# undistro/trivy

Hardware: AMD Instinct MI355X
Metric: GB/s secret-scanned (whole node) at 1/2/4/8 MI355X; findings bit-exact vs CPU (higher is better)
Workload: dtype u8

## Files before the change

### include/tsg_debug.h

```cpp
#ifndef TSG_DEBUG_H
#define TSG_DEBUG_H
#include <stdint.h>
#ifdef __cplusplus
extern "C" {
#endif

int tsg_regex_find_all(const char* pattern, const uint8_t* text, uint64_t n, int submatch,
                       const int64_t* windows, uint32_t n_windows, int64_t* out, uint64_t out_cap,
                       uint64_t* out_len, int32_t* num_cap);

void tsg_debug_regex_engine(int mode);
int tsg_debug_xform(int device, const uint8_t* raw, uint64_t n_bytes, const uint64_t* offsets, uint32_t n_files,
                    const uint8_t* kinds, uint8_t* out, uint64_t out_cap, uint64_t* xoff);
int tsg_debug_classify(int device, const uint8_t* raw, uint64_t n_bytes, const uint64_t* offsets, uint32_t n_files,
                       uint8_t* flags);
int tsg_debug_transform_census(int device, const uint8_t* raw, uint64_t n_bytes, const uint64_t* offsets,
                               uint32_t n_files, const uint8_t* kinds, uint8_t* mark_out);
int tsg_debug_gather_device(int device, const uint8_t* raw, uint64_t n_bytes, const uint64_t* src_off,
                            const uint64_t* dst_off, uint32_t n_files, uint8_t* out);
int tsg_regex_match(const char* pattern, const uint8_t* text, uint64_t n);

int64_t tsg_go_bytes_to_lower(const uint8_t* s, uint64_t n, uint8_t* out, uint64_t out_cap);

struct tsg_global;
// ... 20 lines not shown
                     int32_t* off_lo, int32_t* off_hi);
const char* tsg_debug_keyword(const tsg_compiled* c, uint32_t k);
const void* tsg_debug_anchor_req(const tsg_compiled* c, uint32_t j);
int tsg_debug_filter(const tsg_compiled* c, uint32_t* shape, const uint32_t** reach, const uint32_t** bucket_off,
                     const uint32_t** bucket_items, const void** items, uint32_t* n_items, const uint8_t** item_cls,
                     const uint32_t** classes, double* est_fp);
int tsg_debug_filter_ids(const tsg_compiled* c, const uint32_t** ids, uint32_t* n);
int tsg_debug_filter_core(const tsg_compiled* c, uint32_t out[4]);
const char* tsg_debug_rule_anchor(const tsg_compiled* c, uint32_t i);


int tsg_debug_pool_budget(void);

struct tsg_scanner;
int tsg_debug_scanner_engine(struct tsg_scanner* s, uint64_t out[4]);

int tsg_debug_scanner_gpu_findings(struct tsg_scanner* s, int mode);

int tsg_debug_scanner_fetch(struct tsg_scanner* s, uint64_t stage_bytes, uint64_t direct_bytes);

int tsg_regex_find_all_bounded(const char* pattern, const uint8_t* text, uint64_t true_len, uint64_t lo, uint64_t hi,
                               int submatch, const int64_t* windows, uint32_t n_windows, int64_t* out,
                               uint64_t out_cap, uint64_t* out_len, int32_t* num_cap, int32_t* hit_limit);
int tsg_debug_fetch_windows_plan(const uint64_t* offsets, uint32_t n_files, const void* cands, uint64_t n_cands,
                                 const uint32_t* rule_max_len, uint32_t n_rules, const uint32_t* opts, uint64_t* runs,
                                 uint64_t runs_cap, uint64_t* n_runs, uint64_t* views, uint64_t views_cap,
                                 uint64_t* n_views, uint64_t totals[4]);
int tsg_debug_fetch_windows_device(int device, const uint8_t* arena, uint64_t n_bytes, const uint64_t* offsets,
                                   uint32_t n_files, const void* cands, uint64_t n_cands, uint32_t cand_cap,
                                   const uint32_t* rule_max_len, uint32_t n_rules, const uint32_t* opts,
// ... 16 lines not shown
  uint32_t kw_words;
  uint32_t counters[16];
  uint32_t caps[3];
  uint32_t reserved_;
  uint64_t* hits;        uint64_t hits_cap, n_hits;
  uint32_t* kw;          uint64_t kw_cap, n_kw;
  uint32_t* flags;       uint64_t flags_cap, n_flags;
  uint16_t* nl;          uint64_t nl_cap, n_nl;
  uint32_t* chunk_file;  uint64_t chunk_file_cap, n_chunk_file;
  uint32_t* recs;        uint64_t recs_cap, n_recs;
  void* cands;           uint64_t cands_cap, n_cands;
} tsg_debug_stage_dump;
int tsg_debug_engine_stages(const tsg_compiled* c, int device, const uint8_t* arena, uint64_t n_bytes,
                            const uint64_t* offsets, uint32_t n_files, const uint8_t tail[64],
                            tsg_debug_stage_dump* out);
int tsg_debug_scan_grow(const uint32_t counters[16], const uint32_t fs_counters[6], uint32_t caps[7]);

int tsg_debug_tar_headers(int device, const void* dev_tar, uint64_t n_bytes, uint64_t capacity, uint32_t grid_cap,
                          void* records_out, uint64_t* count_out, double* ms_out);
void tsg_debug_set_tar_capacity(uint64_t records);
struct tsg_analyzer;
struct tsg_tar_index;
struct tsg_device_tar_stats;
int tsg_debug_index_tar_records(struct tsg_analyzer* a, const uint8_t* host_tar, uint64_t n_bytes,
                                const void* records, uint64_t n_records, struct tsg_tar_index** out,
                                struct tsg_device_tar_stats* st);
int tsg_debug_tar_chain(int device, const void* dev_tar, uint64_t n_bytes, uint32_t segment_blocks, uint32_t grid_cap,
                        void* records_out, uint64_t rec_cap, uint64_t* n_records, uint8_t* names_out,
                        uint64_t name_cap, uint64_t* name_bytes, uint64_t* stop_out, uint64_t* candidates_out);
int tsg_debug_tar_walk_last_fallback(const struct tsg_analyzer* a);
// ... 14 lines not shown
```

### trivy_amd/csrc/capi_debug.cpp

```cpp
#include "tsg_debug.h"

#include <algorithm>
#include <atomic>
#include <cstring>
#include <memory>
#include <string>
#include <vector>

#include "capi_internal.h"
#include "census.h"
#include "classify.h"
#include "fetch_host.h"
#include "fetch_windows.h"
#include "filter.h"
#include "goregex.h"
#include "parallel.h"
#include "xform.h"

namespace tsg {
extern std::atomic<int> g_regex_engine;
thread_local std::string g_last_error;
void SetError(const std::string& e) { g_last_error = e; }
}

extern "C" {

const char* tsg_last_error(void) { return tsg::g_last_error.c_str(); }

int tsg_regex_find_all(const char* pattern, const uint8_t* text, uint64_t n, int submatch,
                       const int64_t* windows, uint32_t n_windows, int64_t* out, uint64_t out_cap,
// ... 421 lines not shown
  window_stats->granules = r->win.granules;
  window_stats->runs = r->win.runs;
  window_stats->window_bytes = r->win.window_bytes;
  window_stats->sparse_files = r->win.sparse_files;
  window_stats->whole_files = r->win.whole_files;
  window_stats->fallback_files = r->win.fallback_files;
  window_stats->fallback_bytes = r->win.fallback_bytes;
  window_stats->ms_fallback = r->win.ms_fallback;
  *out = r.release();
  return 0;
}

int tsg_debug_engine_stages(const tsg_compiled* c, int device, const uint8_t* arena, uint64_t n_bytes,
                            const uint64_t* offsets, uint32_t n_files, const uint8_t tail[64],
                            tsg_debug_stage_dump* out) {
  if (!c || !offsets || !tail || !out || (n_bytes && !arena)) {
    tsg::SetError("tsg_debug_engine_stages: NULL argument");
    return -2;
  }
  if (out->struct_size != sizeof(tsg_debug_stage_dump)) {
    tsg::SetError("tsg_debug_engine_stages: unknown tsg_debug_stage_dump.struct_size");
    return -2;
  }
  if (!WinArgsOk("tsg_debug_engine_stages", offsets, n_files, nullptr)) return -2;
  if (offsets[n_files] != n_bytes) {
    tsg::SetError("tsg_debug_engine_stages: offsets must end at n_bytes");
    return -2;
  }
  void *d_arena = nullptr, *d_off = nullptr;
  hipError_t e = hipSetDevice(device);
  auto ok = [&](hipError_t r) {
    if (e == hipSuccess) e = r;
    return e == hipSuccess;
  };
  tsg::StageDump d;
  std::string run_err;
  if (ok(e) && ok(hipMalloc(&d_arena, n_bytes + 64)) && ok(hipMalloc(&d_off, (size_t(n_files) + 1) * 8)) &&
      ok(hipMemcpy(static_cast<uint8_t*>(d_arena) + n_bytes, tail, 64, hipMemcpyHostToDevice)) &&
      (n_bytes == 0 || ok(hipMemcpy(d_arena, arena, n_bytes, hipMemcpyHostToDevice))) &&
      ok(hipMemcpy(d_off, offsets, (size_t(n_files) + 1) * 8, hipMemcpyHostToDevice))) {
    std::unique_ptr<tsg::GpuEngine> eng(new tsg::GpuEngine(c->cr, device));
    std::vector<tsg::Candidate> cands;
    if (!eng->ok() || !eng->Run(static_cast<const uint8_t*>(d_arena), n_bytes, static_cast<const uint64_t*>(d_off),
                                n_files, &cands, nullptr, nullptr, nullptr, &d))
      run_err = eng->error().empty() ? "engine failed" : eng->error();
  }
  for (void* p : {d_arena, d_off})
    if (p) (void)hipFree(p);
  if (e != hipSuccess || !run_err.empty()) {
    tsg::SetError(std::string("tsg_debug_engine_stages: ") + (e != hipSuccess ? hipGetErrorString(e) : run_err.c_str()));
    return -1;
  }
  out->kw_words = d.kw_words;
  static_assert(sizeof(out->counters) == tsg::kScanCtrBytes, "tsg_debug_stage_dump hands out the scan counters whole");
  std::memcpy(out->counters, d.counters, sizeof(out->counters));
  out->caps[0] = d.hit_cap;
  out->caps[1] = d.rec_cap;
  out->caps[2] = d.cand_cap;
  auto put = [](void* dst, uint64_t cap, uint64_t* n, const void* src, size_t count, size_t rec) {
    *n = count;
    const size_t k = size_t(std::min<uint64_t>(cap, count));
    if (dst && k) std::memcpy(dst, src, k * rec);
// ... 33 lines not shown
  std::vector<std::vector<uint64_t>> cols;
  for (uint32_t b = 0; b < 256; b++) {
    std::vector<uint64_t> col(n_groups);
    for (uint32_t g = 0; g < n_groups; g++) col[g] = f->core[size_t(g) * 256 + b];
    if (std::find(cols.begin(), cols.end(), col) == cols.end()) cols.push_back(std::move(col));
  }
  uint32_t most = 0;
  for (uint32_t b = 0; b + 1 < f->bucket_groups.size(); b++) most = std::max(most, f->bucket_groups[b + 1] - f->bucket_groups[b]);
  out[0] = n_groups;
  out[1] = uint32_t(cols.size());
  out[2] = most;
  out[3] = uint32_t(f->hash_keys.size());
  return 0;
}

int tsg_debug_sure_allow(const char* const* patterns, uint32_t n_patterns, const uint8_t* paths, const uint64_t* off,
                         uint32_t n_paths, uint8_t* sure, uint8_t* has_form) {
  std::vector<std::unique_ptr<tsg::Regex>> own;
  std::vector<const tsg::Regex*> res;
  for (uint32_t i = 0; i < n_patterns; i++) {
    std::string err;
    own.push_back(tsg::Regex::Compile(patterns[i], &err));
    if (!own.back()) {
      tsg::SetError(err);
      return -1;
    }
    res.push_back(own.back().get());
  }
  tsg::SureTable t;
  std::vector<uint8_t> form;
// ... 19 lines not shown
```

### trivy_amd/csrc/capi_scanner.cpp

```cpp
#include <pthread.h>
#include <condition_variable>
#include <cstring>
#include <deque>
#include <mutex>
#include <thread>
#include <memory>
#include <string>

#include "capi_internal.h"
#include "filter.h"
#include "scanner.h"
#include "tsg_debug.h"
#include "tsg_scanner.h"

namespace {
class ResultReaper {
 public:
  static ResultReaper& Get() {
    static ResultReaper r;
    return r;
  }
  void Push(tsg_result* r) {
    if (!r) return;
    {
// ... 668 lines not shown
}

int tsg_debug_scanner_engine(tsg_scanner* s, uint64_t out[4]) {
  out[0] = out[1] = out[2] = out[3] = 0;
  if (!s || !s->s || s->s->n_engines() == 0) return -1;
  for (size_t i = 0; i < s->s->n_engines(); i++) {
    const tsg::GpuEngine::HostMemInfo m = s->s->engine_at(i)->host_mem_info();
    out[0] += m.retired_pending;
    out[1] += m.retired_freed;
    out[2] = std::max<uint64_t>(out[2], m.cand_cap);
    out[3] += m.slot_bytes;
  }
  return 0;
}

int tsg_scanner_set_fetch_options(tsg_scanner* s, const tsg_fetch_options* opt) {
  if (!s || !s->s || !opt) {
    tsg::SetError("tsg_scanner_set_fetch_options: NULL argument");
    return -1;
  }
  if (opt->struct_size != TSG_FETCH_OPTIONS_SIZE_V1) {
    tsg::SetError("tsg_scanner_set_fetch_options: tsg_fetch_options.struct_size " + std::to_string(opt->struct_size) +
                  " is not a size this library knows (v1 = " + std::to_string(TSG_FETCH_OPTIONS_SIZE_V1) + ")");
    return -1;
  }
  if (opt->mode > TSG_FETCH_WINDOWS) {
    tsg::SetError("tsg_scanner_set_fetch_options: mode " + std::to_string(opt->mode) +
                  " (0 = files, 1 = windows are the modes)");
    return -1;
  }
// ... 114 lines not shown
```

### trivy_amd/csrc/engine.h

```cpp
#pragma once
#include <hip/hip_runtime.h>

#include <cstdint>
#include <atomic>
#include <condition_variable>
#include <deque>
#include <memory>
#include <string>
#include <mutex>
#include <thread>
#include <vector>

#include "fetch_layout.h"
#include "rules.h"
#include "scan_layout.h"

namespace tsg {

constexpr uint32_t kChunk = 1024;

constexpr uint32_t kCandGateOpen = 1;
constexpr uint32_t kCandFoldFile = 2;
constexpr uint32_t kCandGateValid = 4;
constexpr uint32_t kCandDrop = 8;
// ... 210 lines not shown
  std::atomic<uint64_t> fetch_recent_packed_{0}, fetch_recent_total_{0};
  hipStream_t fetch_stream_ = nullptr;
  hipEvent_t ev_packed_ = nullptr, ev_drained_ = nullptr, ev_run_f_[2] = {};
  void* d_fscratch_ = nullptr; size_t cap_fscratch_ = 0;
  void* d_fstage_ = nullptr; size_t cap_fstage_ = 0;
  void* d_fctr_ = nullptr;
  void* h_run_fctr_ = nullptr;
  void* h_fflags_ = nullptr; size_t cap_h_fflags_ = 0;
  std::unique_ptr<FetchPool> fetch_pool_;

 public:
  struct HostMemInfo {
    uint64_t retired_pending, retired_freed, cand_cap, slot_bytes;
  };
  HostMemInfo host_mem_info();

 private:
  bool Transform(int b, uint32_t nf, const uint8_t** arena, const uint64_t** offsets, uint64_t* n_bytes,
                 std::vector<uint64_t>* xoff, float* ms);
  bool GatherTail(const std::vector<Candidate>& part, uint32_t f0, uint32_t nf, const std::vector<uint64_t>& xoff,
                  const uint64_t* raw_off, const uint8_t* kinds, std::vector<uint64_t>* tail_len, TailOut* tail);
  void DumpItemDiag();
  bool DumpStages(const WorkSet& W, const uint32_t* cnt, uint64_t n_bytes, uint32_t n_files, StageDump* d);
  std::vector<uint8_t> h_items_kind_;
  std::vector<uint32_t> h_items_id_;
  std::string err_;
  int device_ = 0;
  hipStream_t stream_ = nullptr;
  PhaseEvents run_ev_;
  uint32_t diag_mode_ = 0, diag_confirm_ = 0;
  AnchorInfo* d_anchors_ = nullptr;
  RuleGpu* d_rules_ = nullptr;
  uint32_t* d_rule_kw_ = nullptr;
  uint64_t* d_nfa_ = nullptr;
  uint32_t* d_fullscan_rules_ = nullptr;
  uint32_t kw_words_ = 0, n_rules_ = 0, n_fullscan_rules_ = 0;
  std::vector<uint32_t> fullscan_rules_;
  uint32_t* d_reach_ = nullptr;
  uint64_t* d_core_ = nullptr;
  uint32_t* d_group_items_ = nullptr;
  uint32_t* d_bucket_groups_ = nullptr;
  void* d_ftabs_ = nullptr;
  void* d_fold_pairs_ = nullptr;
  void* d_fold_first_ = nullptr;
  uint32_t n_fold_pairs_k_ = 0, n_fold_pairs_s_ = 0, n_fold_cap_k_ = 0, n_fold_cap_s_ = 0;
// ... 86 lines not shown
```

### trivy_amd/csrc/engine.hip

```cpp
#include <chrono>
#include <condition_variable>
#include <mutex>
#include <hip/hip_runtime.h>

#include <algorithm>
#include <cstdlib>
#include <cstdio>
#include <cstring>
#include <string>
#include <pthread.h>

#include <thread>
#include <type_traits>

#include "engine.h"
#include "census.h"
#include "fetch.h"
#include "fetch_host.h"
#include "fetch_windows.h"
#include "xform.h"
#include "filter.h"

namespace tsg {

namespace {

constexpr int kScanThreads = 1024;
constexpr int kScanWaves = kScanThreads / 64;

#define HIP_OK(x)                                                   \
  do {                                                              \
    hipError_t e_ = (x);                                            \
    if (e_ != hipSuccess) {                                         \
      err_ = std::string(#x) + ": " + hipGetErrorString(e_);        \
      return false;                                                 \
    }                                                               \
// ... 74 lines not shown
#define TSG_K1_NLTILES 16
#endif
constexpr int kFNlTiles = TSG_K1_NLTILES;
#ifndef TSG_K1_WGS
#define TSG_K1_WGS 2
#endif
constexpr int kFWgPerCu = TSG_K1_WGS;
#ifndef TSG_K1_GROUPQ
#define TSG_K1_GROUPQ 1
#endif
constexpr uint32_t kFGroup = 8;
#ifndef TSG_K1_READAHEAD
#define TSG_K1_READAHEAD 4
#endif
constexpr uint32_t kFReadAhead = TSG_K1_READAHEAD;
constexpr int kFWindow = 6;
constexpr int kFWords = 4;
constexpr uint32_t kFireBits = 0xFFF00000u;
constexpr uint32_t kNlBits = 0x8888u;
static_assert(kChunk % kFLane == 0 && kChunk / kFLane <= 64, "a newline chunk must be whole lane chunks");
static_assert(kFChunks * kChunk == kFTile && kFChunks == 4, "a tile's newline counts are one u64");


constexpr uint32_t kRunWords = 8;
__host__ __device__ inline uint64_t KeepWords(uint64_t n_tiles) {
  return ((n_tiles + 63) / 64 + kRunWords - 1) / kRunWords * kRunWords;
}

__global__ __launch_bounds__(256) void tile_keep_kernel(const uint64_t* __restrict__ off, uint32_t n_files,
                                                        const uint32_t* __restrict__ chunk_file,
// ... 125 lines not shown
  uint64_t n_bytes;
  const uint2* runs;
  uint32_t* run_info;
  const uint32_t* reach;
  uint32_t diag_mode;
  uint16_t* nl;
  uint32_t* recs;
  uint32_t rec_cap;
  uint32_t* counters;
};

__device__ __forceinline__ uint4 reach_read(const uint8_t* sb, uint32_t w, uint32_t k, uint32_t laneoff) {
  return *reinterpret_cast<const uint4*>(sb + __builtin_amdgcn_perm(w, laneoff, 0x0C0C0000u | ((4u + k) << 8)));
}

__device__ __forceinline__ void reach_apply(const uint4& m, uint32_t* st) {
  asm("v_lshl_or_b32 %0, %1, 4, %2" : "=v"(st[0]) : "v"(st[0]), "v"(m.x));
  asm("v_lshl_or_b32 %0, %1, 4, %2" : "=v"(st[1]) : "v"(st[1]), "v"(m.y));
  asm("v_lshl_or_b32 %0, %1, 4, %2" : "=v"(st[2]) : "v"(st[2]), "v"(m.z));
  asm("v_lshl_or_b32 %0, %1, 4, %2" : "=v"(st[3]) : "v"(st[3]), "v"(m.w));
}

__device__ __forceinline__ uint32_t nl_count4(uint32_t w) {
  const uint32_t a = ((w ^ 0x0A0A0A0Au) & 0x7F7F7F7Fu) + 0x7F7F7F7Fu;
  return __popc(~(a | w) & 0x80808080u);
}

__device__ __forceinline__ uint32_t word_of(uint4 v, uint32_t i) {
  return i < 2 ? (i == 0 ? v.x : v.y) : (i == 2 ? v.z : v.w);
}

__device__ __forceinline__ void load_reach_lds(uint8_t* s_reach, const uint32_t* reach, uint32_t copies, int tid,
                                               int nthreads) {
  for (uint32_t i = tid; i < 256 * copies; i += nthreads) {
    const uint32_t b = i / copies;
    reinterpret_cast<uint4*>(s_reach)[i] = reinterpret_cast<const uint4*>(reach)[b];
  }
}

template <bool kRuns>
__global__ __launch_bounds__(kScanThreads, 8) void filter_kernel(FilterParams P) {
  __shared__ __attribute__((aligned(16))) uint8_t s_reach[65536];
  __shared__ uint32_t s_queue[kScanWaves * kFQueue];
  __shared__ uint64_t s_nl[kScanWaves * kFNlTiles];
  const int tid = threadIdx.x;
  load_reach_lds(s_reach, P.reach, 16, tid, blockDim.x);
  __syncthreads();
  const uint32_t lane = tid & 63;
  const uint32_t wave = __builtin_amdgcn_readfirstlane(uint32_t(tid) >> 6);
  const uint32_t laneoff = (lane & 15) * 16;
  uint32_t* Q = s_queue + wave * kFQueue;
  uint64_t* NL = s_nl + wave * kFNlTiles;
  uint32_t nl_slots = 0;
  uint32_t qn = 0;
  const uint64_t n_tiles = (P.n_bytes + kFTile - 1) / kFTile;
  const uint64_t n_waves = uint64_t(gridDim.x) * kScanWaves;
  const uint64_t wid = uint64_t(blockIdx.x) * kScanWaves + wave;
  const uint2* __restrict__ RUNS = kRuns ? P.runs : nullptr;
  auto uni = [](uint32_t v) { return uint32_t(__builtin_amdgcn_readfirstlane(v)); };
  const uint64_t n_kept = RUNS ? uint64_t(uni(P.run_info[kSkKept])) : n_tiles;
  const bool tail_kept = RUNS ? uni(P.run_info[kSkTailKept]) != 0 : true;
  const uint64_t per = n_kept / n_waves, extra = n_kept % n_waves;
  const uint64_t k_begin = wid * per + (wid < extra ? wid : extra);
  const uint64_t k_end = k_begin + per + (wid < extra ? 1 : 0);
  uint32_t run = 0;
  uint64_t run_k1 = n_kept;
  uint64_t t_begin = k_begin;
  uint32_t runs_walked = 1;
  if (RUNS && k_begin < k_end) {
    uint32_t lo = 0, hi = uni(P.run_info[kSkRuns]);
    while (hi - lo > 1) {
      const uint32_t mid = (lo + hi) >> 1;
      if (uni(RUNS[mid].y) <= k_begin) lo = mid;
      else hi = mid;
    }
    run = lo;
    const uint2 r0 = RUNS[lo];
    t_begin = uint64_t(uni(r0.x)) + (k_begin - uni(r0.y));
    run_k1 = uni(RUNS[lo + 1].y);
// ... 5 lines not shown
    pre_x = __builtin_amdgcn_readfirstlane(pv.x);
    pre_y = __builtin_amdgcn_readfirstlane(pv.y);
  };
  if (k_begin < k_end && t_begin > 0) load_pre(t_begin);
  auto next_tile = [&](uint64_t k1, uint64_t tcur, bool* nr) -> uint64_t {
    if (k1 < run_k1) {
      *nr = false;
      return tcur + 1;
    }
    run++;
    runs_walked++;
    run_k1 = uni(RUNS[run + 1].y);
    *nr = true;
    return uni(RUNS[run].x);
  };
  auto load_tile = [&](uint4* dst, uint64_t tt) {
    const uint64_t b0 = tt * kFTile + uint64_t(lane) * kFLane;
    const uint8_t* lp = P.arena + (b0 < P.n_bytes ? b0 : 0);
#pragma unroll
    for (int j = 0; j < kFBlocks; j++) dst[j] = load16(lp + 16 * j);
  };
  auto flush = [&]() {
    uint32_t base = 0;
    if (lane == 0) base = atomicAdd(&P.counters[kCtRecs], qn);
    base = __builtin_amdgcn_readfirstlane(base);
    for (uint32_t i = lane; i < qn; i += 64) {
      if (base + i < P.rec_cap) P.recs[base + i] = Q[i];
      else P.counters[kCtRecOvf] = 1;
    }
    qn = 0;
  };
#if TSG_K1_GROUPQ
  uint32_t fl_acc = 0;
  uint32_t grp_n = 0;
  uint64_t grp_t0 = 0;
  auto compact = [&]() {
    const uint32_t cnt = __popc(fl_acc);
    uint32_t incl = cnt;
    incl += uint32_t(__builtin_amdgcn_update_dpp(0, int(incl), 0x111, 0xF, 0xF, true));
    incl += uint32_t(__builtin_amdgcn_update_dpp(0, int(incl), 0x112, 0xF, 0xF, true));
    incl += uint32_t(__builtin_amdgcn_update_dpp(0, int(incl), 0x114, 0xF, 0xF, true));
    incl += uint32_t(__builtin_amdgcn_update_dpp(0, int(incl), 0x118, 0xF, 0xF, true));
    incl += uint32_t(__builtin_amdgcn_update_dpp(0, int(incl), 0x142, 0xA, 0xF, false));
    incl += uint32_t(__builtin_amdgcn_update_dpp(0, int(incl), 0x143, 0xC, 0xF, false));
    const uint32_t total = __builtin_amdgcn_readlane(incl, 63);
    if (total) {
      if (qn + total > kFQueue) flush();
      const uint32_t rec0 = __builtin_amdgcn_readfirstlane(uint32_t(grp_t0 * (kFTile / 16))) + lane * kFBlocks;
      uint32_t m = fl_acc;
      if (total <= kFQueue) {
        uint32_t at = qn + incl - cnt;
        while (m) {
          const uint32_t b = uint32_t(__builtin_ctz(m));
          m &= m - 1;
          Q[at++] = rec0 + ((b >> 2) << 8) + (b & 3u);
        }
        qn += total;
      } else {
        uint32_t base = 0;
        if (lane == 0) base = atomicAdd(&P.counters[kCtRecs], total);
        uint32_t at = __builtin_amdgcn_readfirstlane(base) + incl - cnt;
        while (m) {
          const uint32_t b = uint32_t(__builtin_ctz(m));
          m &= m - 1;
          if (at < P.rec_cap) P.recs[at] = rec0 + ((b >> 2) << 8) + (b & 3u);
          else P.counters[kCtRecOvf] = 1;
          at++;
        }
      }
    }
    fl_acc = 0;
    grp_n = 0;
  };
#endif
  auto flush_nl = [&](uint64_t t_last) {
    wave_sync();
    uint32_t l = lane;
    asm volatile("" : "+v"(l));
    if (l < nl_slots) {
      const uint64_t tt = t_last - uint64_t(nl_slots - 1 - l);
      reinterpret_cast<uint64_t*>(P.nl)[tt] = NL[l];
    }
    nl_slots = 0;
  };
  auto tile = [&](uint4* cur, uint64_t tt, auto tail_tag) {
    constexpr bool kTail = decltype(tail_tag)::value;
    if (kTail) {
      const uint64_t b0 = tt * kFTile + uint64_t(lane) * kFLane;
#pragma unroll
      for (int j = 0; j < kFBlocks; j++) {
        const uint64_t p = b0 + 16 * j;
        uint32_t wd[4] = {cur[j].x, cur[j].y, cur[j].z, cur[j].w};
#pragma unroll
        for (int q = 0; q < 4; q++) {
          const uint64_t wp = p + 4 * q;
          if (wp >= P.n_bytes) wd[q] = 0;
          else if (wp + 4 > P.n_bytes) wd[q] &= (1u << (8 * (P.n_bytes - wp))) - 1u;
        }
        cur[j] = make_uint4(wd[0], wd[1], wd[2], wd[3]);
      }
    }
    const uint32_t p0 = uint32_t(__builtin_amdgcn_update_dpp(int(pre_x), int(cur[kFBlocks - 1].z), 0x138, 0xF, 0xF,
                                                             false));
    const uint32_t p1 = uint32_t(__builtin_amdgcn_update_dpp(int(pre_y), int(cur[kFBlocks - 1].w), 0x138, 0xF, 0xF,
                                                             false));
    pre_x = __builtin_amdgcn_readlane(cur[kFBlocks - 1].z, 63);
    pre_y = __builtin_amdgcn_readlane(cur[kFBlocks - 1].w, 63);
    uint32_t flagged = 0, nl = 0;
    if (P.diag_mode < 2) {
      uint32_t st[kFWords] = {~0u, ~0u, ~0u, ~0u};
      reach_apply(reach_read(s_reach, p0, 3, laneoff), st);
#pragma unroll
      for (uint32_t k = 0; k < 4; k++) reach_apply(reach_read(s_reach, p1, k, laneoff), st);
#pragma unroll
      for (int j = 0; j < kFBlocks; j++) {
        const uint32_t wd[4] = {cur[j].x, cur[j].y, cur[j].z, cur[j].w};
        uint32_t acc = ~0u;
#pragma unroll
        for (uint32_t g = 0; g < 16; g += kFReadAhead) {
          uint4 m[kFReadAhead];
#pragma unroll
          for (uint32_t q = 0; q < kFReadAhead; q++)
            m[q] = reach_read(s_reach, wd[(g + q) >> 2], (g + q) & 3, laneoff);
#pragma unroll
          for (uint32_t q = 0; q < kFReadAhead; q++) {
            const uint32_t k = g + q;
            reach_apply(m[q], st);
            if (k % 3 == 2 || k == 15) acc &= st[0] & st[1] & st[2] & st[3];
            if (k % 4 == 3) nl += __popc(~st[3] & kNlBits);
          }
        }
        flagged |= uint32_t((acc | ~kFireBits) != ~0u) << j;
      }
    } else {
#pragma unroll
      for (int j = 0; j < kFBlocks; j++)
        nl += nl_count4(cur[j].x) + nl_count4(cur[j].y) + nl_count4(cur[j].z) + nl_count4(cur[j].w);
    }
    {
    nl += uint32_t(__builtin_amdgcn_update_dpp(0, int(nl), 0x111, 0xF, 0xF, true));
    nl += uint32_t(__builtin_amdgcn_update_dpp(0, int(nl), 0x112, 0xF, 0xF, true));
    nl += uint32_t(__builtin_amdgcn_update_dpp(0, int(nl), 0x114, 0xF, 0xF, true));
    nl += uint32_t(__builtin_amdgcn_update_dpp(0, int(nl), 0x118, 0xF, 0xF, true));
    static_assert(kChunk / kFLane == 16, "one newline chunk per DPP row");
    static_assert(kFTile / 16 == 256, "a tile's records: 256 blocks");
    if ((lane & 15) == 15) reinterpret_cast<uint16_t*>(NL + nl_slots)[lane >> 4] = uint16_t(nl);
    if (++nl_slots == kFNlTiles) flush_nl(tt);
    }
#if TSG_K1_GROUPQ
    if (grp_n == 0) grp_t0 = tt;
    fl_acc |= flagged << (4 * grp_n);
    grp_n++;
#else
    const uint32_t rec0 = uint32_t(tt * (kFTile / 16)) + lane * kFBlocks;
#pragma unroll
    for (int j = 0; j < kFBlocks; j++) {
      const bool fj = (flagged >> j) & 1u;
      const uint64_t m = __ballot(fj);
      if (m) {
        if (qn + 64 > kFQueue) flush();
        const uint32_t below =
// ... 4 lines not shown
    }
#endif
  };
  auto flush_due = [&]() {
#if TSG_K1_GROUPQ
    if (grp_n == kFGroup) compact();
#endif
    if (qn >= kFFlushAt) flush();
  };
  using Full = std::false_type;
  if constexpr (!kRuns) {
    const uint64_t t_end = k_end;
    const uint64_t t_full = t_end < P.n_bytes / kFTile ? t_end : P.n_bytes / kFTile;
    uint64_t t = t_begin;
    if (t < t_full) load_tile(bufA, t);
    while (t < t_full) {
      flush_due();
      load_tile(bufB, t + 1 < t_full ? t + 1 : t);
      tile(bufA, t, Full());
      t++;
      if (t >= t_full) break;
      flush_due();
      load_tile(bufA, t + 1 < t_full ? t + 1 : t);
      tile(bufB, t, Full());
      t++;
    }
    if (t < t_end) {
      flush_due();
      load_tile(bufA, t);
      tile(bufA, t, std::true_type());
      t++;
    }
#if TSG_K1_GROUPQ
    if (grp_n) compact();
#endif
    if (qn) flush();
    if (nl_slots) flush_nl(t - 1);
    return;
  }
  const bool partial = (P.n_bytes % kFTile) != 0 && tail_kept;
  const uint64_t k_full = (partial && k_end == n_kept && k_end > k_begin) ? k_end - 1 : k_end;
  uint64_t k = k_begin, t = t_begin, t_prev = t_begin;
  bool nr_cur = false;
  auto run_boundary = [&]() {
#if TSG_K1_GROUPQ
    if (grp_n) compact();
#endif
    if (nl_slots) flush_nl(t_prev);
  };
  auto step = [&](uint4* cur, uint4* nxt) {
    if (nr_cur) run_boundary();
    flush_due();
    uint64_t tn = t;
    bool nr_n = false;
    if (k + 1 < k_end) tn = next_tile(k + 1, t, &nr_n);
    if (nr_cur) load_pre(t);
    load_tile(nxt, k + 1 < k_full ? tn : t);
    tile(cur, t, Full());
    t_prev = t;
    t = tn;
    nr_cur = nr_n;
    k++;
  };
  if (k < k_full) load_tile(bufA, t);
  while (k < k_full) {
    step(bufA, bufB);
    if (k >= k_full) break;
    step(bufB, bufA);
  }
  if (k < k_end) {
    if (nr_cur) run_boundary();
    flush_due();
    if (nr_cur) load_pre(t);
    load_tile(bufA, t);
    tile(bufA, t, std::true_type());
    t_prev = t;
    k++;
  }
#if TSG_K1_GROUPQ
  if (grp_n) compact();
#endif
  if (qn) flush();
  if (nl_slots) flush_nl(t_prev);
// ... 1581 lines not shown
        return hipHostMalloc(&p, n, hipHostMallocDefault) == hipSuccess ? p : nullptr;
      },
      [this](void* p) { RetireHost(p); }));
  if (hipSetDevice(device) != hipSuccess) {
    err_ = "hipSetDevice failed (no HIP device?)";
    return;
  }
  if (hipStreamCreateWithFlags(&stream_, hipStreamNonBlocking) != hipSuccess ||
      hipStreamCreateWithFlags(&copy_stream_, hipStreamNonBlocking) != hipSuccess) {
    err_ = "hipStreamCreate failed";
    return;
  }
  {
    if (const char* e = std::getenv("TSG_OVERLAP_K0")) overlap_k0_ = std::atoi(e) != 0;
    if (const char* e = std::getenv("TSG_READBACK_STREAM")) readback_stream_ = std::atoi(e) != 0;
    int lo = 0, hi = 0;
    if (hipDeviceGetStreamPriorityRange(&lo, &hi) != hipSuccess) lo = hi = 0;
    bool ok = hipStreamCreateWithPriority(&aux_stream_, hipStreamNonBlocking, hi) == hipSuccess &&
              hipStreamCreateWithFlags(&rb_stream_, hipStreamNonBlocking) == hipSuccess;
    for (WorkSet& W : sets_)
      ok = ok && hipEventCreateWithFlags(&W.free_ev, hipEventDisableTiming) == hipSuccess &&
           hipEventCreateWithFlags(&W.k0_done, hipEventDisableTiming) == hipSuccess;
    ok = ok && run_ev_.Create();
    ok = ok && hipEventCreateWithFlags(&k2_done_, hipEventDisableTiming) == hipSuccess;
    if (!ok) {
      err_ = "hipStreamCreate / hipEventCreate failed (K0 and read-back streams)";
      return;
    }
  }
  for (auto& e : ev_copied_) hipEventCreateWithFlags(&e, hipEventDisableTiming);
// ... 1449 lines not shown
    HIP_OK(hipGetLastError());
  }
  HIP_OK(hipEventRecord(E.ev_k0[1], k0s));
  if (k0_aux) {
    HIP_OK(hipEventRecord(W.k0_done, aux_stream_));
    W.k0_rec = true;
    HIP_OK(hipEventRecord(E.ev[kEvStart], stream_));
    if (d_item_diag_) HIP_OK(hipMemsetAsync(d_item_diag_, 0, 8 * std::max<size_t>(n_fitems_, 1), stream_));
    HIP_OK(hipStreamWaitEvent(stream_, W.k0_done, 0));
  }
  const FilterParams fp = KernelArgs::Filter(*this, W, d_arena, n_bytes, skip);
  uint32_t f_grid =
      uint32_t(std::max<uint64_t>(1, std::min<uint64_t>((f_tiles + kScanWaves - 1) / kScanWaves, 256 * kFWgPerCu)));
  if (k1_grid_cap_) f_grid = std::min(f_grid, k1_grid_cap_);
  HIP_OK(hipEventRecord(E.ev[kEvK1], stream_));
  if (skip) filter_kernel<true><<<f_grid, kScanThreads, 0, stream_>>>(fp);
  else filter_kernel<false><<<f_grid, kScanThreads, 0, stream_>>>(fp);
  HIP_OK(hipGetLastError());
  HIP_OK(hipEventRecord(E.ev[kEvK2], stream_));
  ConfirmParams cp = KernelArgs::Confirm(*this, W, d_arena, n_bytes, d_offsets);
  static const bool k2_pack = std::getenv("TSG_K2_PACK") && std::atoi(std::getenv("TSG_K2_PACK")) != 0;
  if (k2_pack && diag_mode_ == 0) {
    if (!Ensure(&d_wins_, &cap_wins_, size_t(caps_.rec) * 64)) return false;
    pack_windows_kernel<<<8192, 256, 0, stream_>>>(d_arena, n_bytes, static_cast<const uint32_t*>(d_recs_), caps_.rec,
                                                   W.counters, static_cast<uint8_t*>(d_wins_));
    HIP_OK(hipGetLastError());
    HIP_OK(hipEventRecord(E.ev[kEvK2], stream_));
    cp.wins = static_cast<const uint8_t*>(d_wins_);
  }
  if (diag_mode_ == 0) {
    if (lds_tabs_)
      confirm_kernel<true><<<2048 * 256 / kCThreads, kCThreads, c_lds_bytes_, stream_>>>(cp);
// ... 386 lines not shown
```

Measured before the change: 2842.

## Add OR-form reach table for K1 filter with single-buffer refill

Adds an alternative K1 filter formulation that rearranges the per-byte reach table into an OR-form layout. Window state is then combined with or3 and bitop3 instructions across position pairs instead of the serial shift-or state update. The OR-form path is on by default, with an environment variable to select the old shift-or form. It also drops the double-buffered tile loads and refills the current buffer block-by-block during compute, which lowers register pressure but may expose load latency. Debug APIs are added to query the active form and to run the engine stages with a skip mask.

```diff
diff --git a/include/tsg_debug.h b/include/tsg_debug.h
--- a/include/tsg_debug.h
+++ b/include/tsg_debug.h
@@ -58,6 +58,8 @@
 
 struct tsg_scanner;
 int tsg_debug_scanner_engine(struct tsg_scanner* s, uint64_t out[4]);
+int tsg_debug_scanner_k1_form(struct tsg_scanner* s);
+int tsg_debug_filter_orform(const tsg_compiled* c, uint32_t out[1024]);
 
 int tsg_debug_scanner_gpu_findings(struct tsg_scanner* s, int mode);
 
@@ -104,6 +106,9 @@
 int tsg_debug_engine_stages(const tsg_compiled* c, int device, const uint8_t* arena, uint64_t n_bytes,
                             const uint64_t* offsets, uint32_t n_files, const uint8_t tail[64],
                             tsg_debug_stage_dump* out);
+int tsg_debug_engine_stages_skip(const tsg_compiled* c, int device, const uint8_t* arena, uint64_t n_bytes,
+                                 const uint64_t* offsets, uint32_t n_files, const uint8_t tail[64],
+                                 const uint8_t* skip, tsg_debug_stage_dump* out);
 int tsg_debug_scan_grow(const uint32_t counters[16], const uint32_t fs_counters[6], uint32_t caps[7]);
 
 int tsg_debug_tar_headers(int device, const void* dev_tar, uint64_t n_bytes, uint64_t capacity, uint32_t grid_cap,
diff --git a/trivy_amd/csrc/capi_debug.cpp b/trivy_amd/csrc/capi_debug.cpp
--- a/trivy_amd/csrc/capi_debug.cpp
+++ b/trivy_amd/csrc/capi_debug.cpp
@@ -14,6 +14,7 @@
 #include "fetch_windows.h"
 #include "filter.h"
 #include "goregex.h"
+#include "k1_orform.h"
 #include "parallel.h"
 #include "xform.h"
 
@@ -465,6 +466,12 @@
 int tsg_debug_engine_stages(const tsg_compiled* c, int device, const uint8_t* arena, uint64_t n_bytes,
                             const uint64_t* offsets, uint32_t n_files, const uint8_t tail[64],
                             tsg_debug_stage_dump* out) {
+  return tsg_debug_engine_stages_skip(c, device, arena, n_bytes, offsets, n_files, tail, nullptr, out);
+}
+
+int tsg_debug_engine_stages_skip(const tsg_compiled* c, int device, const uint8_t* arena, uint64_t n_bytes,
+                                 const uint64_t* offsets, uint32_t n_files, const uint8_t tail[64],
+                                 const uint8_t* skip, tsg_debug_stage_dump* out) {
   if (!c || !offsets || !tail || !out || (n_bytes && !arena)) {
     tsg::SetError("tsg_debug_engine_stages: NULL argument");
     return -2;
@@ -478,7 +485,7 @@
     tsg::SetError("tsg_debug_engine_stages: offsets must end at n_bytes");
     return -2;
   }
-  void *d_arena = nullptr, *d_off = nullptr;
+  void *d_arena = nullptr, *d_off = nullptr, *d_skip = nullptr;
   hipError_t e = hipSetDevice(device);
   auto ok = [&](hipError_t r) {
     if (e == hipSuccess) e = r;
@@ -489,14 +496,18 @@
   if (ok(e) && ok(hipMalloc(&d_arena, n_bytes + 64)) && ok(hipMalloc(&d_off, (size_t(n_files) + 1) * 8)) &&
       ok(hipMemcpy(static_cast<uint8_t*>(d_arena) + n_bytes, tail, 64, hipMemcpyHostToDevice)) &&
       (n_bytes == 0 || ok(hipMemcpy(d_arena, arena, n_bytes, hipMemcpyHostToDevice))) &&
-      ok(hipMemcpy(d_off, offsets, (size_t(n_files) + 1) * 8, hipMemcpyHostToDevice))) {
+      ok(hipMemcpy(d_off, offsets, (size_t(n_files) + 1) * 8, hipMemcpyHostToDevice)) &&
+      (!skip || n_files == 0 ||
+       (ok(hipMalloc(&d_skip, n_files)) && ok(hipMemcpy(d_skip, skip, n_files, hipMemcpyHostToDevice))))) {
     std::unique_ptr<tsg::GpuEngine> eng(new tsg::GpuEngine(c->cr, device));
     std::vector<tsg::Candidate> cands;
+    tsg::SkipIn sk;
+    sk.d_skip = static_cast<const uint8_t*>(d_skip);
     if (!eng->ok() || !eng->Run(static_cast<const uint8_t*>(d_arena), n_bytes, static_cast<const uint64_t*>(d_off),
-                                n_files, &cands, nullptr, nullptr, nullptr, &d))
+                                n_files, &cands, nullptr, nullptr, d_skip ? &sk : nullptr, &d))
       run_err = eng->error().empty() ? "engine failed" : eng->error();
   }
-  for (void* p : {d_arena, d_off})
+  for (void* p : {d_arena, d_off, d_skip})
     if (p) (void)hipFree(p);
   if (e != hipSuccess || !run_err.empty()) {
     tsg::SetError(std::string("tsg_debug_engine_stages: ") + (e != hipSuccess ? hipGetErrorString(e) : run_err.c_str()));
@@ -560,6 +571,13 @@
   return 0;
 }
 
+int tsg_debug_filter_orform(const tsg_compiled* c, uint32_t out[1024]) {
+  const auto* f = c->cr.filter.get();
+  if (!f || f->n_buckets != 16 || f->n_words != 4 || f->window > 6 || f->reach.size() != 256 * 4) return -1;
+  for (uint32_t b = 0; b < 256; b++) tsg::OrFormRow(&f->reach[size_t(b) * 4], out + size_t(b) * 4);
+  return 0;
+}
+
 int tsg_debug_sure_allow(const char* const* patterns, uint32_t n_patterns, const uint8_t* paths, const uint64_t* off,
                          uint32_t n_paths, uint8_t* sure, uint8_t* has_form) {
   std::vector<std::unique_ptr<tsg::Regex>> own;
diff --git a/trivy_amd/csrc/capi_scanner.cpp b/trivy_amd/csrc/capi_scanner.cpp
--- a/trivy_amd/csrc/capi_scanner.cpp
+++ b/trivy_amd/csrc/capi_scanner.cpp
@@ -706,6 +706,11 @@
   return 0;
 }
 
+int tsg_debug_scanner_k1_form(tsg_scanner* s) {
+  if (!s || !s->s || s->s->n_engines() == 0) return -1;
+  return s->s->engine_at(0)->k1_or_form() ? 1 : 0;
+}
+
 int tsg_scanner_set_fetch_options(tsg_scanner* s, const tsg_fetch_options* opt) {
   if (!s || !s->s || !opt) {
     tsg::SetError("tsg_scanner_set_fetch_options: NULL argument");
diff --git a/trivy_amd/csrc/engine.h b/trivy_amd/csrc/engine.h
--- a/trivy_amd/csrc/engine.h
+++ b/trivy_amd/csrc/engine.h
@@ -248,6 +248,7 @@
     uint64_t retired_pending, retired_freed, cand_cap, slot_bytes;
   };
   HostMemInfo host_mem_info();
+  bool k1_or_form() const { return k1_or_; }
 
  private:
   bool Transform(int b, uint32_t nf, const uint8_t** arena, const uint64_t** offsets, uint64_t* n_bytes,
@@ -263,6 +264,7 @@
   hipStream_t stream_ = nullptr;
   PhaseEvents run_ev_;
   uint32_t diag_mode_ = 0, diag_confirm_ = 0;
+  bool k1_or_ = true;
   AnchorInfo* d_anchors_ = nullptr;
   RuleGpu* d_rules_ = nullptr;
   uint32_t* d_rule_kw_ = nullptr;
diff --git a/trivy_amd/csrc/engine.hip b/trivy_amd/csrc/engine.hip
--- a/trivy_amd/csrc/engine.hip
+++ b/trivy_amd/csrc/engine.hip
@@ -20,6 +20,7 @@
 #include "fetch_windows.h"
 #include "xform.h"
 #include "filter.h"
+#include "k1_orform.h"
 
 namespace tsg {
 
@@ -124,6 +125,13 @@
 #define TSG_K1_READAHEAD 4
 #endif
 constexpr uint32_t kFReadAhead = TSG_K1_READAHEAD;
+#ifndef TSG_K1_OR_READAHEAD
+#define TSG_K1_OR_READAHEAD 4
+#endif
+#ifndef TSG_K1_OR_WHOLE_TAIL
+#define TSG_K1_OR_WHOLE_TAIL 0
+#endif
+constexpr uint32_t kFReadAheadOr = TSG_K1_OR_READAHEAD;
 constexpr int kFWindow = 6;
 constexpr int kFWords = 4;
 constexpr uint32_t kFireBits = 0xFFF00000u;
@@ -279,6 +287,12 @@
   return *reinterpret_cast<const uint4*>(sb + __builtin_amdgcn_perm(w, laneoff, 0x0C0C0000u | ((4u + k) << 8)));
 }
 
+__device__ __forceinline__ uint4 reach_read_whole(const uint8_t* sb, uint32_t w, uint32_t k, uint32_t laneoff) {
+  uint4 r = reach_read(sb, w, k, laneoff);
+  asm volatile("" : "+v"(r.x), "+v"(r.y), "+v"(r.z), "+v"(r.w));
+  return r;
+}
+
 __device__ __forceinline__ void reach_apply(const uint4& m, uint32_t* st) {
   asm("v_lshl_or_b32 %0, %1, 4, %2" : "=v"(st[0]) : "v"(st[0]), "v"(m.x));
   asm("v_lshl_or_b32 %0, %1, 4, %2" : "=v"(st[1]) : "v"(st[1]), "v"(m.y));
@@ -303,19 +317,48 @@
   }
 }
 
-template <bool kRuns>
+__device__ __forceinline__ void load_orform_lds(uint8_t* s_reach, const uint32_t* reach, int tid, int nthreads) {
+  for (uint32_t i = tid; i < 256 * 4; i += nthreads) {
+    const uint32_t b = i >> 2;
+    const uint4 r = reinterpret_cast<const uint4*>(reach)[b];
+    const uint32_t in[4] = {r.x, r.y, r.z, r.w};
+    uint32_t w[4];
+    OrFormRow(in, w);
+#pragma unroll
+    for (uint32_t c = 0; c < 4; c++)
+      reinterpret_cast<uint4*>(s_reach)[b * 16 + (i & 3) * 4 + c] = make_uint4(w[0], w[1], w[2], w[3]);
+  }
+}
+
+__device__ __forceinline__ uint32_t or3_keep(uint32_t a, uint32_t b, uint32_t c) {
+  uint32_t h;
+  asm("v_or3_b32 %0, %1, %2, %3" : "=v"(h) : "v"(a), "v"(b), "v"(c));
+  return h;
+}
+__device__ __forceinline__ uint32_t and_or_keep(uint32_t acc, uint32_t a, uint32_t b) {
+  asm("v_bitop3_b32 %0, %1, %2, %3 bitop3:0xe0" : "=v"(acc) : "v"(acc), "v"(a), "v"(b));
+  return acc;
+}
+
+template <bool kRuns, bool kOr>
 __global__ __launch_bounds__(kScanThreads, 8) void filter_kernel(FilterParams P) {
   __shared__ __attribute__((aligned(16))) uint8_t s_reach[65536];
   __shared__ uint32_t s_queue[kScanWaves * kFQueue];
   __shared__ uint64_t s_nl[kScanWaves * kFNlTiles];
   const int tid = threadIdx.x;
-  load_reach_lds(s_reach, P.reach, 16, tid, blockDim.x);
+  if constexpr (kOr) load_orform_lds(s_reach, P.reach, tid, blockDim.x);
+  else load_reach_lds(s_reach, P.reach, 16, tid, blockDim.x);
   __syncthreads();
   const uint32_t lane = tid & 63;
   const uint32_t wave = __builtin_amdgcn_readfirstlane(uint32_t(tid) >> 6);
   const uint32_t laneoff = (lane & 15) * 16;
   uint32_t* Q = s_queue + wave * kFQueue;
   uint64_t* NL = s_nl + wave * kFNlTiles;
+  auto ln = [&]() {
+    uint32_t l = lane;
+    if constexpr (kOr) asm volatile("" : "+v"(l));
+    return l;
+  };
   uint32_t nl_slots = 0;
   uint32_t qn = 0;
   const uint64_t n_tiles = (P.n_bytes + kFTile - 1) / kFTile;
@@ -326,8 +369,12 @@
   const uint64_t n_kept = RUNS ? uint64_t(uni(P.run_info[kSkKept])) : n_tiles;
   const bool tail_kept = RUNS ? uni(P.run_info[kSkTailKept]) != 0 : true;
   const uint64_t per = n_kept / n_waves, extra = n_kept % n_waves;
-  const uint64_t k_begin = wid * per + (wid < extra ? wid : extra);
-  const uint64_t k_end = k_begin + per + (wid < extra ? 1 : 0);
+  auto uni64 = [&](uint64_t v) {
+    if constexpr (kOr) return uint64_t(uni(uint32_t(v))) | uint64_t(uni(uint32_t(v >> 32))) << 32;
+    else return v;
+  };
+  const uint64_t k_begin = uni64(wid * per + (wid < extra ? wid : extra));
+  const uint64_t k_end = uni64(k_begin + per + (wid < extra ? 1 : 0));
   uint32_t run = 0;
   uint64_t run_k1 = n_kept;
   uint64_t t_begin = k_begin;
@@ -363,17 +410,21 @@
     *nr = true;
     return uni(RUNS[run].x);
   };
+  auto lane_ptr = [&](uint64_t tt) -> const uint8_t* {
+    const uint64_t b0 = tt * kFTile + uint64_t(ln()) * kFLane;
+    return P.arena + (b0 < P.n_bytes ? b0 : 0);
+  };
   auto load_tile = [&](uint4* dst, uint64_t tt) {
-    const uint64_t b0 = tt * kFTile + uint64_t(lane) * kFLane;
-    const uint8_t* lp = P.arena + (b0 < P.n_bytes ? b0 : 0);
+    const uint8_t* lp = lane_ptr(tt);
 #pragma unroll
     for (int j = 0; j < kFBlocks; j++) dst[j] = load16(lp + 16 * j);
   };
   auto flush = [&]() {
     uint32_t base = 0;
-    if (lane == 0) base = atomicAdd(&P.counters[kCtRecs], qn);
+    const uint32_t l = ln();
+    if (l == 0) base = atomicAdd(&P.counters[kCtRecs], qn);
     base = __builtin_amdgcn_readfirstlane(base);
-    for (uint32_t i = lane; i < qn; i += 64) {
+    for (uint32_t i = l; i < qn; i += 64) {
       if (base + i < P.rec_cap) P.recs[base + i] = Q[i];
       else P.counters[kCtRecOvf] = 1;
     }
@@ -395,7 +446,8 @@
     const uint32_t total = __builtin_amdgcn_readlane(incl, 63);
     if (total) {
       if (qn + total > kFQueue) flush();
-      const uint32_t rec0 = __builtin_amdgcn_readfirstlane(uint32_t(grp_t0 * (kFTile / 16))) + lane * kFBlocks;
+      const uint32_t l = ln();
+      const uint32_t rec0 = __builtin_amdgcn_readfirstlane(uint32_t(grp_t0 * (kFTile / 16))) + l * kFBlocks;
       uint32_t m = fl_acc;
       if (total <= kFQueue) {
         uint32_t at = qn + incl - cnt;
@@ -407,7 +459,7 @@
         qn += total;
       } else {
         uint32_t base = 0;
-        if (lane == 0) base = atomicAdd(&P.counters[kCtRecs], total);
+        if (l == 0) base = atomicAdd(&P.counters[kCtRecs], total);
         uint32_t at = __builtin_amdgcn_readfirstlane(base) + incl - cnt;
         while (m) {
           const uint32_t b = uint32_t(__builtin_ctz(m));
@@ -432,8 +484,9 @@
     }
     nl_slots = 0;
   };
-  auto tile = [&](uint4* cur, uint64_t tt, auto tail_tag) {
+  auto tile = [&](uint4* cur, uint64_t tt, auto tail_tag, const uint8_t* nxt = nullptr) {
     constexpr bool kTail = decltype(tail_tag)::value;
+    constexpr bool kRefill = kOr && !kTail;
     if (kTail) {
       const uint64_t b0 = tt * kFTile + uint64_t(lane) * kFLane;
 #pragma unroll
@@ -456,7 +509,48 @@
     pre_x = __builtin_amdgcn_readlane(cur[kFBlocks - 1].z, 63);
     pre_y = __builtin_amdgcn_readlane(cur[kFBlocks - 1].w, 63);
     uint32_t flagged = 0, nl = 0;
-    if (P.diag_mode < 2) {
+    if (kOr && P.diag_mode < 2) {
+      const uint32_t laneoff = (ln() & 15) * 16;
+      constexpr uint32_t kRA = kFReadAheadOr;
+      static_assert(kRA % 2 == 0 && 16 % kRA == 0, "positions are combined in pairs");
+      uint32_t xh[4], yh[2], hprev;
+      {
+        auto row = [&](uint32_t w, uint32_t k) { return reach_read_whole(s_reach, w, k, laneoff); };
+        const uint4 r5 = row(p0, 3), r4 = row(p1, 0), r3 = row(p1, 1), r2 = row(p1, 2), r1 = row(p1, 3);
+        hprev = or3_keep(r5.x, r3.y, r1.z);
+        xh[0] = r4.x, xh[1] = r3.x, xh[2] = r2.x, xh[3] = r1.x;
+        yh[0] = r2.y, yh[1] = r1.y;
+      }
+#pragma unroll
+      for (int j = 0; j < kFBlocks; j++) {
+        const uint32_t wd[4] = {cur[j].x, cur[j].y, cur[j].z, cur[j].w};
+        uint32_t acc = ~0u;
+#pragma unroll
+        for (uint32_t g = 0; g < 16; g += kRA) {
+          uint4 m[kRA];
+#pragma unroll
+          for (uint32_t q = 0; q < kRA; q++) {
+            if (TSG_K1_OR_WHOLE_TAIL && j == kFBlocks - 1 && g + q >= 12) m[q] = reach_read_whole(s_reach, wd[(g + q) >> 2], (g + q) & 3, laneoff);
+            else m[q] = reach_read(s_reach, wd[(g + q) >> 2], (g + q) & 3, laneoff);
+          }
+#pragma unroll
+          for (uint32_t q = 0; q < kRA; q += 2) {
+            const uint32_t k = g + q;
+            const uint32_t h0 = or3_keep(xh[k & 3], yh[0], m[q].z);
+            const uint32_t h1 = or3_keep(xh[(k + 1) & 3], yh[1], m[q + 1].z);
+            xh[k & 3] = m[q].x, xh[(k + 1) & 3] = m[q + 1].x;
+            yh[0] = m[q].y, yh[1] = m[q + 1].y;
+            const uint32_t hi = __builtin_amdgcn_perm(h1, h0, 0x07060302u);
+            const uint32_t lo = __builtin_amdgcn_perm(h0, hprev, 0x05040100u);
+            acc = and_or_keep(acc, hi, lo);
+            nl += m[q].w + m[q + 1].w;
+            hprev = h1;
+          }
+        }
+        flagged |= uint32_t(acc != ~0u) << j;
+        if constexpr (kRefill) cur[j] = load16(nxt + 16 * j);
+      }
+    } else if (P.diag_mode < 2) {
       uint32_t st[kFWords] = {~0u, ~0u, ~0u, ~0u};
       reach_apply(reach_read(s_reach, p0, 3, laneoff), st);
 #pragma unroll
@@ -483,8 +577,10 @@
       }
     } else {
 #pragma unroll
-      for (int j = 0; j < kFBlocks; j++)
+      for (int j = 0; j < kFBlocks; j++) {
         nl += nl_count4(cur[j].x) + nl_count4(cur[j].y) + nl_count4(cur[j].z) + nl_count4(cur[j].w);
+        if constexpr (kRefill) cur[j] = load16(nxt + 16 * j);
+      }
     }
     {
     nl += uint32_t(__builtin_amdgcn_update_dpp(0, int(nl), 0x111, 0xF, 0xF, true));
@@ -493,7 +589,8 @@
     nl += uint32_t(__builtin_amdgcn_update_dpp(0, int(nl), 0x118, 0xF, 0xF, true));
     static_assert(kChunk / kFLane == 16, "one newline chunk per DPP row");
     static_assert(kFTile / 16 == 256, "a tile's records: 256 blocks");
-    if ((lane & 15) == 15) reinterpret_cast<uint16_t*>(NL + nl_slots)[lane >> 4] = uint16_t(nl);
+    const uint32_t l = ln();
+    if ((l & 15) == 15) reinterpret_cast<uint16_t*>(NL + nl_slots)[l >> 4] = uint16_t(nl);
     if (++nl_slots == kFNlTiles) flush_nl(tt);
     }
 #if TSG_K1_GROUPQ
@@ -528,16 +625,24 @@
     const uint64_t t_full = t_end < P.n_bytes / kFTile ? t_end : P.n_bytes / kFTile;
     uint64_t t = t_begin;
     if (t < t_full) load_tile(bufA, t);
-    while (t < t_full) {
-      flush_due();
-      load_tile(bufB, t + 1 < t_full ? t + 1 : t);
-      tile(bufA, t, Full());
-      t++;
-      if (t >= t_full) break;
-      flush_due();
-      load_tile(bufA, t + 1 < t_full ? t + 1 : t);
-      tile(bufB, t, Full());
-      t++;
+    if constexpr (kOr) {
+      while (t < t_full) {
+        flush_due();
+        tile(bufA, t, Full(), lane_ptr(t + 1 < t_full ? t + 1 : t));
+        t++;
+      }
+    } else {
+      while (t < t_full) {
+        flush_due();
+        load_tile(bufB, t + 1 < t_full ? t + 1 : t);
+        tile(bufA, t, Full());
+        t++;
+        if (t >= t_full) break;
+        flush_due();
+        load_tile(bufA, t + 1 < t_full ? t + 1 : t);
+        tile(bufB, t, Full());
+        t++;
+      }
     }
     if (t < t_end) {
       flush_due();
@@ -553,7 +658,7 @@
     return;
   }
   const bool partial = (P.n_bytes % kFTile) != 0 && tail_kept;
-  const uint64_t k_full = (partial && k_end == n_kept && k_end > k_begin) ? k_end - 1 : k_end;
+  const uint64_t k_full = uni64((partial && k_end == n_kept && k_end > k_begin) ? k_end - 1 : k_end);
   uint64_t k = k_begin, t = t_begin, t_prev = t_begin;
   bool nr_cur = false;
   auto run_boundary = [&]() {
@@ -569,18 +674,26 @@
     bool nr_n = false;
     if (k + 1 < k_end) tn = next_tile(k + 1, t, &nr_n);
     if (nr_cur) load_pre(t);
-    load_tile(nxt, k + 1 < k_full ? tn : t);
-    tile(cur, t, Full());
+    if constexpr (kOr) {
+      tile(cur, t, Full(), lane_ptr(k + 1 < k_full ? tn : t));
+    } else {
+      load_tile(nxt, k + 1 < k_full ? tn : t);
+      tile(cur, t, Full());
+    }
     t_prev = t;
     t = tn;
     nr_cur = nr_n;
     k++;
   };
   if (k < k_full) load_tile(bufA, t);
-  while (k < k_full) {
-    step(bufA, bufB);
-    if (k >= k_full) break;
-    step(bufB, bufA);
+  if constexpr (kOr) {
+    while (k < k_full) step(bufA, bufA);
+  } else {
+    while (k < k_full) {
+      step(bufA, bufB);
+      if (k >= k_full) break;
+      step(bufB, bufA);
+    }
   }
   if (k < k_end) {
     if (nr_cur) run_boundary();
@@ -2192,6 +2305,14 @@
   {
     if (const char* e = std::getenv("TSG_OVERLAP_K0")) overlap_k0_ = std::atoi(e) != 0;
     if (const char* e = std::getenv("TSG_READBACK_STREAM")) readback_stream_ = std::atoi(e) != 0;
+    if (const char* e = std::getenv("TSG_K1_FORM")) {
+      if (std::strcmp(e, "or") == 0) k1_or_ = true;
+      else if (std::strcmp(e, "shiftor") == 0) k1_or_ = false;
+      else {
+        err_ = std::string("TSG_K1_FORM=") + e + " (or, shiftor are the forms)";
+        return;
+      }
+    }
     int lo = 0, hi = 0;
     if (hipDeviceGetStreamPriorityRange(&lo, &hi) != hipSuccess) lo = hi = 0;
     bool ok = hipStreamCreateWithPriority(&aux_stream_, hipStreamNonBlocking, hi) == hipSuccess &&
@@ -3671,8 +3792,13 @@
       uint32_t(std::max<uint64_t>(1, std::min<uint64_t>((f_tiles + kScanWaves - 1) / kScanWaves, 256 * kFWgPerCu)));
   if (k1_grid_cap_) f_grid = std::min(f_grid, k1_grid_cap_);
   HIP_OK(hipEventRecord(E.ev[kEvK1], stream_));
-  if (skip) filter_kernel<true><<<f_grid, kScanThreads, 0, stream_>>>(fp);
-  else filter_kernel<false><<<f_grid, kScanThreads, 0, stream_>>>(fp);
+  if (k1_or_) {
+    if (skip) filter_kernel<true, true><<<f_grid, kScanThreads, 0, stream_>>>(fp);
+    else filter_kernel<false, true><<<f_grid, kScanThreads, 0, stream_>>>(fp);
+  } else {
+    if (skip) filter_kernel<true, false><<<f_grid, kScanThreads, 0, stream_>>>(fp);
+    else filter_kernel<false, false><<<f_grid, kScanThreads, 0, stream_>>>(fp);
+  }
   HIP_OK(hipGetLastError());
   HIP_OK(hipEventRecord(E.ev[kEvK2], stream_));
   ConfirmParams cp = KernelArgs::Confirm(*this, W, d_arena, n_bytes, d_offsets);
diff --git a/trivy_amd/csrc/k1_orform.h b/trivy_amd/csrc/k1_orform.h
--- /dev/null
+++ b/trivy_amd/csrc/k1_orform.h
@@ -0,0 +1,22 @@
+#pragma once
+#include <cstdint>
+
+#include "filter.h"
+
+namespace tsg {
+
+TSG_HOST_DEVICE inline void OrFormRow(const uint32_t reach[4], uint32_t out[4]) {
+  for (uint32_t k = 0; k < 3; k++) {
+    uint32_t w = 0;
+    for (uint32_t h = 0; h < 2; h++) {
+      const uint32_t s = 2 * k + h;
+      uint32_t m = 0;
+      for (uint32_t r = 0; r < 4; r++) m |= ((reach[r] >> (4 * s)) & 0xFu) << (4 * r);
+      w |= m << (16 * h);
+    }
+    out[k] = w;
+  }
+  out[3] = (~reach[3] >> 3) & 1u;
+}
+
+}
```

After: 3154, median of 6. 1.11x the previous value.
